# youmi-zym/TemporalStereo

Measured on AMD Instinct MI355X. Metric: stereo pairs/sec, FlyingThings3D 540x960 D=192 (aggregation hot path), higher is better.
Workload: dtype f32

## Files before the change

include/ts_hip.h:

```cpp
#ifndef TS_HIP_H
#define TS_HIP_H

#include <stddef.h>
#include <stdint.h>

#ifdef __cplusplus
extern "C" {
#endif

#define TS_OK 0
#define TS_ERR_NULL (-1)
#define TS_ERR_SHAPE (-2)
#define TS_ERR_UNSUPPORTED (-3)
#define TS_ERR_ALIGN (-4)

int ts_version(void);
const char* ts_last_error_string(void);

size_t ts_block_cost_workspace_bytes(int B, int C, int H, int W, int D, int scales);

int ts_block_cost_int_fwd(const float* left, const float* right, float* out, void* workspace,
                          int B, int C, int H, int W, int D, int scales, void* stream);

int ts_block_cost_sampled_fwd(const float* left, const float* right, const float* disp, float* out,
// ... 132 lines not shown
                          long long color_aug_stride, void* stream);
int ts_intrinsics_pyramid_fwd(const void* K_norm, int is_fp64, int B, int kh, int kw, int S, float* K, float* inv_K, void* stream);
int ts_disp_u16_decode_fwd(const void* raw, int B, int H, int W, float scale, float* disp, void* valid, void* stream);

#define TS_AUGMENT_ROW_INTS 96
#define TS_AUGMENT_MAX_RECTS 4
#define TS_AUGMENT_GAMMA 1
size_t ts_frames_augment_workspace_bytes(int B, int Hs, int Ws);
int ts_frames_augment_fwd(const void* left, const void* right, int B, int Hs, int Ws, int flags, float mean0, float mean1,
                          float mean2, float std0, float std1, float std2, int H, int W, const int* table, float* color_l,
                          float* color_r, long long color_stride, float* color_aug_l, float* color_aug_r,
                          long long color_aug_stride, void* workspace, size_t workspace_bytes, void* stream);
int ts_disp_u16_window_fwd(const void* raw, int B, int Hs, int Ws, int H, int W, const int* table, float scale, float* disp,
                           void* valid, void* stream);

int ts_topk_softargmax_fwd(const float* cost, const float* sample, const float* offset, float* disp,
                           float* topk_disp, float* topk_cost, int* topk_index,
                           int B, int D, int H, int W, int k, void* stream);

int ts_topk_softargmax_bwd(const float* topk_disp, const float* topk_cost, const int* topk_index,
                           const float* disp, const float* grad_disp, const float* grad_topk_disp,
                           const float* grad_topk_cost, float* grad_cost, float* grad_sample,
                           int B, int D, int H, int W, int k, void* stream);

int ts_softargmin_fwd(const float* cost, const float* sample, float* disp, float temperature,
                      int normalize, int B, int D, int H, int W, void* stream);

int ts_softargmin_bwd(const float* cost, const float* sample, const float* disp, const float* grad_disp,
                      float* grad_cost, float* grad_sample, float temperature, int normalize,
                      int B, int D, int H, int W, void* stream);

int ts_argmax_select_fwd(const float* cost, const float* sample, float* disp, int* index,
                         int B, int D, int H, int W, void* stream);

int ts_softsplat_sum_fwd(const float* input, const float* flow, float* output,
                         int B, int C, int H, int W, void* stream);
int ts_softsplat_sum_fwd_deterministic(const float* input, const float* flow, float* output, void* workspace,
                                       int B, int C, int H, int W, void* stream);
int ts_softsplat_sum_bwd_input(const float* flow, const float* grad_output, float* grad_input,
                               int B, int C, int H, int W, void* stream);
int ts_softsplat_sum_bwd_flow(const float* input, const float* flow, const float* grad_output,
                              float* grad_flow, int B, int C, int H, int W, void* stream);
size_t ts_softsplat_softmax_workspace_bytes(int B, int C, int H, int W);
int ts_softsplat_softmax_fwd(const float* input, const float* flow, const float* metric, float* output,
                             void* workspace, int B, int C, int H, int W, void* stream);
int ts_project_to_3d_fwd(const float* depth, const float* K, const float* inv_K, const float* T,
// ... 181 lines not shown
```

temporalstereo_amd/_lib.py:

```python
import ctypes
import os
import threading

_HERE = os.path.dirname(os.path.abspath(__file__))
LIB_PATH = os.path.join(_HERE, "libts_hip.so")

_lock = threading.Lock()
_lib = None

c_f32p = ctypes.c_void_p
c_ptr = ctypes.c_void_p
c_int = ctypes.c_int
c_size = ctypes.c_size_t
c_float = ctypes.c_float

SIGNATURES = {
    "ts_version": (c_int, []),
    "ts_last_error_string": (ctypes.c_char_p, []),
    "ts_block_cost_workspace_bytes": (c_size, [c_int] * 6),
    "ts_block_cost_int_fwd": (c_int, [c_f32p, c_f32p, c_f32p, c_ptr] + [c_int] * 6 + [c_ptr]),
    "ts_block_cost_sampled_fwd": (c_int, [c_f32p, c_f32p, c_f32p, c_f32p, c_ptr] + [c_int] * 6 + [c_ptr]),
    "ts_block_cost_sampled_warped_fwd": (c_int, [c_f32p, c_f32p, c_f32p, c_f32p, c_ptr] + [c_int] * 6 + [c_ptr]),
    "ts_block_cost_sampled_corr_fwd": (c_int, [c_f32p, c_f32p, c_f32p, c_f32p, c_ptr] + [c_int] * 6 + [c_ptr]),
    "ts_block_cost_corr_split_supported": (c_int, [c_int] * 2),
# ... 11 lines not shown
    "ts_cat_fms_fwd": (c_int, [c_f32p] * 4 + [c_int] * 5 + [c_ptr]),
    "ts_inverse_warp_3d_fwd": (c_int, [c_f32p] * 3 + [c_int] * 5 + [c_ptr]),
    "ts_dif_fms_workspace_bytes": (c_size, []),
    "ts_dif_fms_fwd": (c_int, [c_f32p] * 4 + [c_ptr] + [c_int] * 5 + [c_ptr]),
    "ts_correlation_fwd": (c_int, [c_f32p] * 3 + [c_int] * 7 + [c_ptr]),
    "ts_correlation_bwd": (c_int, [c_f32p] * 6 + [c_int] * 7 + [c_ptr]),
    "ts_block_cost_bwd_workspace_bytes": (c_size, [c_int] * 6),
    "ts_block_cost_int_bwd": (c_int, [c_f32p] * 5 + [c_ptr] + [c_int] * 6 + [c_ptr]),
    "ts_block_cost_sampled_bwd": (c_int, [c_f32p] * 7 + [c_ptr] + [c_int] * 6 + [c_ptr]),
    "ts_block_cost_sampled_warped_bwd": (c_int, [c_f32p] * 7 + [c_ptr] + [c_int] * 6 + [c_ptr]),
    "ts_calib_stream": (c_int, [c_int, c_ptr, c_ptr, c_size, c_ptr]),
    "ts_candidates_in_range_fwd": (c_int, [c_f32p] * 3 + [c_int] * 5 + [c_ptr]),
    "ts_candidates_in_range_bwd": (c_int, [c_f32p] * 5 + [c_int] * 5 + [c_ptr]),
    "ts_offset_head_fwd": (c_int, [c_f32p] * 2 + [ctypes.c_longlong, c_float, c_ptr]),
    "ts_offset_head_bwd": (c_int, [c_f32p] * 3 + [ctypes.c_longlong, c_float, c_ptr]),
    "ts_space_to_depth2_fwd": (c_int, [c_f32p] * 2 + [c_int] * 4 + [c_ptr]),
    "ts_deconv2d_k4s2_weight_to_conv3": (c_int, [c_f32p] * 2 + [c_int] * 3 + [c_ptr]),
    "ts_deconv2d_k4s2_wgrad_from_conv3": (c_int, [c_f32p] * 2 + [c_int] * 2 + [c_ptr]),
    "ts_bn_fold_many": (c_int, [c_ptr, c_int, c_float, c_ptr]),
    "ts_clip_rmsprop_workspace_bytes": (c_size, [c_int]),
    "ts_clip_rmsprop_step": (c_int, [c_ptr, c_int] + [c_float] * 4 + [c_ptr, c_size, c_ptr]),
    "ts_topk_softargmax_fwd": (c_int, [c_f32p] * 7 + [c_int] * 5 + [c_ptr]),
    "ts_topk_softargmax_bwd": (c_int, [c_f32p] * 9 + [c_int] * 5 + [c_ptr]),
    "ts_softargmin_fwd": (c_int, [c_f32p] * 3 + [c_float, c_int] + [c_int] * 4 + [c_ptr]),
    "ts_softargmin_bwd": (c_int, [c_f32p] * 6 + [c_float, c_int] + [c_int] * 4 + [c_ptr]),
    "ts_argmax_select_fwd": (c_int, [c_f32p] * 4 + [c_int] * 4 + [c_ptr]),
    "ts_bn_workspace_bytes": (c_size, [c_int, c_int, ctypes.c_longlong]),
    "ts_channel_splice_fwd": (c_int, [c_f32p] * 3 + [c_int] * 3 + [ctypes.c_longlong] * 4 + [c_ptr]),
    "ts_bn_sync_merge": (c_int, [c_f32p, c_int, c_int] + [c_f32p] * 4 + [c_float, c_f32p, c_ptr]),
    "ts_bn_train_fwd": (c_int, [c_f32p] * 5 + [c_float, c_ptr] + [c_f32p] * 3 + [c_ptr, c_int, c_int] + [ctypes.c_longlong] * 5 +
                        [c_float, c_int, c_ptr]),
    "ts_bn_train_bwd": (c_int, [c_f32p] * 9 + [c_ptr, c_int, c_int] + [ctypes.c_longlong] * 5 + [c_float, c_int, c_float, c_ptr]),
    "ts_bn_stats_fwd": (c_int, [c_f32p] * 5 + [c_float, c_ptr, c_ptr, c_int, c_int] + [ctypes.c_longlong] * 3 + [c_ptr]),
    "ts_bn_apply_act_fwd": (c_int, [c_f32p] * 6 + [c_int, c_int] + [ctypes.c_longlong] * 5 + [c_float, c_int, c_ptr]),
    "ts_bn_act_bwd_reduce": (c_int, [c_f32p] * 8 + [c_ptr, c_int, c_int] + [ctypes.c_longlong] * 5 + [c_float, c_int, c_ptr]),
    "ts_bn_act_bwd_apply": (c_int, [c_f32p] * 9 + [c_int, c_int] + [ctypes.c_longlong] * 5 + [c_float, c_int, c_int, c_float, c_ptr]),
    "ts_wasserstein_loss_workspace_bytes": (c_size, [c_int] * 3),
    "ts_wasserstein_loss_fwd": (c_int, [c_f32p] * 6 + [c_ptr] + [c_int] * 6 + [c_float, c_float, c_int, c_ptr]),
    "ts_wasserstein_loss_bwd": (c_int, [c_f32p] * 7 + [c_int] * 5 + [c_float, c_float, c_ptr]),
    "ts_disp_smooth_l1_workspace_bytes": (c_size, [c_int] * 3),
    "ts_disp_smooth_l1_fwd": (c_int, [c_f32p] * 3 + [c_ptr] + [c_int] * 5 + [c_float, c_float, c_ptr]),
    "ts_disp_smooth_l1_bwd": (c_int, [c_f32p] * 5 + [c_int] * 5 + [c_float, c_float, c_ptr]),
    "ts_disp_metrics_workspace_bytes": (c_size, [c_int] * 3),
    "ts_disp_metrics_fwd": (c_int, [c_f32p] * 4 + [c_int] * 9 + [c_f32p] * 2 + [c_int] * 3 + [c_float, c_float, c_int, c_f32p, c_ptr, c_ptr]),
    "ts_disp_render_workspace_bytes": (c_size, [c_int] * 3),
    "ts_disp_render_fwd": (c_int, [c_f32p] * 4 + [c_int] * 6 + [c_float] + [c_ptr] * 4 + [c_f32p, c_ptr, c_ptr]),
# ... 68 lines not shown
    "ts_resize_bilinear_pair_fwd": (c_int, [c_f32p] * 4 + [c_int] * 6 + [c_float, c_float, c_ptr]),
    "ts_range_candidates_fwd": (c_int, [c_f32p] * 4 + [c_int] * 3 + [c_float, c_int, c_int, c_ptr]),
    "ts_project_to_3d_fwd": (c_int, [c_f32p] * 7 + [c_int] * 6 + [c_float, c_ptr]),
    "ts_reproject_memory_workspace_bytes": (c_size, [c_int] * 5),
    "ts_reproject_memory_fwd": (c_int, [c_f32p, ctypes.c_longlong, c_int, c_int, c_f32p, c_f32p, c_int, c_f32p, c_int, c_int,
                                        c_f32p, c_int, c_f32p, c_f32p, c_f32p, c_float, c_float, c_f32p, c_f32p, c_f32p,
                                        c_ptr, c_int, c_int, c_int, c_ptr]),
    "ts_resize3d_add_act_bwd": (c_int, [c_f32p] * 5 + [c_int] * 9 + [c_ptr]),
    "ts_pool3d5_avgmax_bwd": (c_int, [c_f32p] * 4 + [c_int] * 5 + [c_ptr]),
    "ts_merge_candidates_bwd": (c_int, [c_f32p] * 5 + [c_int] * 5 + [c_ptr]),
    "ts_copy_rows_fwd": (c_int, [c_f32p] * 2 + [ctypes.c_longlong] * 4 + [c_ptr]),
    "ts_plan_create": (c_ptr, []),
    "ts_plan_destroy": (None, [c_ptr]),
    "ts_plan_length": (c_int, [c_ptr]),
    "ts_plan_add_call": (c_int, [c_ptr, ctypes.c_char_p, ctypes.POINTER(ctypes.c_ulonglong), c_int]),
    "ts_plan_run": (c_int, [c_ptr]),
    "ts_stream_fork": (c_int, [c_ptr, c_ptr]),
    "ts_event_record": (c_int, [c_int, c_ptr]),
    "ts_event_wait": (c_int, [c_int, c_ptr]),
}

_QUERIES = frozenset(n for n in SIGNATURES if n.endswith("_bytes") or n.startswith("ts_plan_") or
                     n.endswith("_split_supported") or
                     n in ("ts_version", "ts_last_error_string", "ts_conv_cout_pad", "ts_conv3d_hw_x6_supported", "ts_conv3d_hw_x6s_supported", "ts_peer_max_floats", "ts_peer_max_ranks",
                           "ts_peer_alloc", "ts_peer_open", "ts_peer_close", "ts_peer_free", "ts_peer_status", "ts_peer_status_async",
                           "ts_peer_set_timeout_ms", "ts_peer_reset", "ts_bn_set_small_elems",
                           "ts_conv_wgrad_defer", "ts_conv_wgrad_pending", "ts_conv_wgrad_take"))


def lib():
    rec = getattr(_tls, "recorder", None)
    if rec is not None:
        return rec.proxy
    return _real_lib()


def _real_lib():
    global _lib
    if _lib is None:
        with _lock:
            if _lib is None:
                if not os.path.exists(LIB_PATH):
                    raise RuntimeError(
                        "temporalstereo_amd: %s is missing -- build it with "
                        "`python -m temporalstereo_amd.build` (there is no fallback path)" % LIB_PATH)
                handle = ctypes.CDLL(LIB_PATH)
                for name, (res, args) in SIGNATURES.items():
# ... 115 lines not shown
```

temporalstereo_amd/aggregation/native.py:

```python
import os
import time

import torch
import torch.nn as nn

from .. import _lib
from .. import functional as TF

ACT_NONE, ACT_SILU, ACT_RELU, ACT_TANH_OFFSET, ACT_HEAD_PAIR = 0, 1, 2, 3, 4


def _stream():
    return _lib.current_stream_handle()


_PAR = {"on": False, "aux": None, "kinds": frozenset(__import__("os").environ.get("TS_BRANCHES", "hourglass").split(","))}


def _aux_stream():
    return _PAR["aux"]


_STAGE_CAP = int(os.environ.get("TS_STAGE_CHUNK_CAP", "8"))

# ... 414 lines not shown
        i2b, i2c = _strides5(split)
    assert Cin == f.cin, (Cin, f.cin)
    Dout = 2 * Din if transposed else (Din + 2 * padding - dilation * (k - 1) - 1) // stride + 1
    if out is None:
        out = torch.empty((B, f.cout, Dout, H, W), device=x.device, dtype=torch.float32)
    ib, ic = _strides5(x)
    ob, oc = _strides5(out)
    if split is not None:
        rc = _lib.lib().ts_conv3d_d_split_fwd(_lib.ptr(x), _lib.ptr(split), _lib.ptr(f.w), _lib.ptr(f.scale), _lib.ptr(f.shift),
                                              _lib.ptr(out), B, Cin, Cs, f.cout, Din, H, W, k, stride, dilation, padding,
                                              int(transposed), f.act if act is None else act, float(act_param),
                                              ib, ic, i2b, i2c, ob, oc, _stream())
        _lib.check(rc, "ts_conv3d_d_split_fwd")
        return out
    rc = _lib.lib().ts_conv3d_d_fwd(_lib.ptr(x), _lib.ptr(f.w), _lib.ptr(f.scale), _lib.ptr(f.shift), _lib.ptr(out),
                                    B, Cin, f.cout, Din, H, W, k, stride, dilation, padding, int(transposed),
                                    f.act if act is None else act, float(act_param), ib, ic, ob, oc, _stream())
    _lib.check(rc, "ts_conv3d_d_fwd")
    return out


FUSED_K1 = os.environ.get("TS_FUSED_K1", "1") != "0"
SPLIT_INPUT = os.environ.get("TS_SPLIT_INPUT", "1") != "0"


def block_cost_corr(left, right, disp, scales):
    return TF.block_cost_corr(left, right, disp, scales)


def conv_hw_warp(corr, f, q, disp, base, dilation=1):
    B, Cc, D, H, W = corr.shape
    assert Cc == f.cin, (Cc, f.cin)
    out = torch.empty((B, f.cout, D, H, W), device=corr.device, dtype=torch.float32)
    ib, ic = _strides5(corr)
    ob, oc = _strides5(out)
    wsb = TF._q("ts_conv3d_hw_warp_workspace_bytes", B, f.cout, D, H, W)
    ws = torch.empty(wsb, device=corr.device, dtype=torch.uint8)
    rc = _lib.lib().ts_conv3d_hw_warp_fwd(_lib.ptr(corr), _lib.ptr(f.w), _lib.ptr(f.scale), _lib.ptr(f.shift), _lib.ptr(out),
                                          _lib.ptr(q), _lib.ptr(disp), _lib.ptr(base), B, Cc, f.cout, D, H, W, dilation, f.act, 0.0,
                                          ib, ic, ob, oc, base.stride(0) if base is not None else 0, _lib.ptr(ws), wsb, _stream())
    _lib.check(rc, "ts_conv3d_hw_warp_fwd")
    return out


def resize_add_act(a, add, size, act=ACT_SILU):
    B, C, Da, Ha, Wa = a.shape
# ... 130 lines not shown
        f = object.__new__(Folded)
        f.cin, f.cout, f.kind, f.act, f.kshape = 2 * C, 2, "hw", ACT_HEAD_PAIR, self.c1.kshape
        pad = int(_lib.lib().ts_conv_cout_pad(2))
        f.w = torch.zeros(2 * C, self.c1.w.shape[1], pad, device=self.c1.w.device, dtype=torch.float32)
        f.w[:C, :, 0] = self.c1.w[:, :, 0]
        f.w[C:, :, 1] = self.o1.w[:, :, 0]
        f.scale = torch.ones(pad, device=f.w.device); f.shift = torch.zeros(pad, device=f.w.device)
        f.scale[0], f.scale[1] = self.c1.scale[0], self.o1.scale[0]
        f.shift[0], f.shift[1] = self.c1.shift[0], self.o1.shift[0]
        f._tape = _TAPE
        if _TAPE is not None:
            for k, (m, g) in enumerate(((mod.cost_head[1], self.c1), (mod.off_head[1], self.o1))):
                _TAPE.layout(f.w[k * C:(k + 1) * C], m.weight.detach(), False, col0=k)
                _TAPE.fold(f.scale[k:k + 1], f.shift[k:k + 1], m.bias, getattr(m, "norm", None), 1)
        self.pair = f

    def __call__(self, x):
        y = conv_d(x, self.co0, 3, 1, 1, 1)
        B, _, D, H, W = y.shape
        both = torch.empty((2, B, D, H, W), device=y.device, dtype=torch.float32)
        conv_hw(y, self.pair, out=both.permute(1, 0, 2, 3, 4), act_param=self.delta)
        return both[0], both[1]


class ConvexUp:

    def __init__(self, mod):
        self.r, self.k = mod.upscale_factor, mod.window_size
        if self.k != 3:
            raise NotImplementedError("window_size != 3")
        self.m0 = Folded(mod.mask[0].weight.unsqueeze(2), mod.mask[0].bias, mod.mask[1], ACT_SILU, False, "hw")
        w3 = mod.mask[3].weight
        self.m3 = Folded(w3.reshape(w3.shape[0], w3.shape[1], 1, 1, 1), mod.mask[3].bias, None, ACT_NONE, False, "d")

    def mask(self, feat):
        return conv_d(conv_hw(feat.unsqueeze(2), self.m0), self.m3, 1)

    def with_candidates(self, feat, disp, m, rng, extra_front=0):
        B, _, H, W = disp.shape
        if m is None:
            m = self.mask(feat)
        Ho, Wo = H * self.r, W * self.r
        out = torch.empty((B, 1, Ho, Wo), device=disp.device, dtype=torch.float32)
        low, high = torch.empty_like(out), torch.empty_like(out)
        cand = torch.empty((B, extra_front + 5, Ho, Wo), device=disp.device, dtype=torch.float32)
        disp = _lib.contiguous(disp)
# ... 78 lines not shown
        samp = torch.empty((B, Dm, H, W), device=vol.device, dtype=torch.float32)
        x0 = cat4[:, :C]
        vb, vc = _strides5(vol); ob, oc = _strides5(x0)
        rc = _lib.lib().ts_merge_candidates_fwd(_lib.ptr(vol), _lib.ptr(samples), _lib.ptr(mem_s), _lib.ptr(mem_c),
                                                _lib.ptr(self.past_w), _lib.ptr(self.past_scale), _lib.ptr(self.past_shift),
                                                _lib.ptr(samp), _lib.ptr(x0), B, C, D0, K, H, W, vb, vc, ob, oc, _stream())
        _lib.check(rc, "ts_merge_candidates_fwd")
        return cat4, samp

    def fuse(self, cat4):
        C = self.C
        x0 = cat4[:, :C]
        if not self.fusion:
            return x0
        br = Branch("pool")
        with br:
            pool5(x0, cat4[:, 2 * C:3 * C], cat4[:, 3 * C:])
        conv_d(x0, self.conv5, 5, 1, 1, 2, out=cat4[:, C:2 * C])
        br.join()
        return self.fuse_conv(cat4)

    def merge_fuse_predict(self, vol, samples, prev_info, feat, resize_memory, mask=None, next_range=None):
        cat4, samp = self.merge(vol, samples, prev_info, resize_memory)
        cost, off = self.heads(self.fuse(cat4))
        disp, _, _ = TF.topk_softargmax(cost, samp, off, k=self.topk)
        if callable(mask):
            mask = mask()
        if next_range is not None:
            return self.up.with_candidates(feat, disp, mask, *next_range), cost, off, samp
        return self.up(feat, disp, mask), cost, off, samp


class NativeCoarse(_MergingLevel):
    def early(self, left, right):
        return self.init3d(TF.block_cost(left, right, int(self.mod.num_sample), self.scales))

    def __call__(self, left, right, prev_info, mask=None, next_range=None, vol=None):
        if vol is None:
            vol = self.early(left, right)
        return self.merge_fuse_predict(vol, None, prev_info, left, resize_memory=True, mask=mask, next_range=next_range)


class NativeFine(_MergingLevel):
    def __init__(self, mod):
        super().__init__(mod)
        self.split_reference_half()

    def early(self, left, right, ds, terms=None):
# ... 107 lines not shown
        lcat, cat2, B, H, W = st
        f = self._c2d(self._c2d(lcat.unsqueeze(2), self.fuse[0], 1), self.fuse[1], 1).squeeze(2)
        self._deconv(_lib.contiguous(f), self.deconv4, cat2, cat2.stride(0))
        g = _lib.contiguous(self._c2d(cat2.unsqueeze(2), self.concat, 1).squeeze(2))
        mask = torch.empty((B, 9, 4 * H, 4 * W), device=lcat.device, dtype=torch.float32)
        self._deconv(g, self.deconv2, mask, mask.stride(0))
        return mask

    def early(self, both, lterm, ds):
        B = both.shape[0] // 2
        lcat, rcat = both.pair() if isinstance(both, SplitBoth) else (both[:B], both[B:])
        lt, rt = lterm
        if rt is not None:
            return self.init3d_from(self.first_layer_fused(lcat, rcat, ds, lt, rt))
        return self.init3d(TF.block_cost_warped(lcat, rcat, ds, self.scales), lt)

    def __call__(self, both, mask_lterm, ds, prev_info, vol=None):
        B = both.shape[0] // 2
        H, W = both.shape[-2:]
        mask, lterm = mask_lterm
        mask = mask() if callable(mask) else mask
        if vol is None:
            vol = self.early(both, lterm, ds)
        cost, off = self.heads(vol)
        disp, mem_s, mem_c = TF.topk_softargmax(cost, ds, off, k=self.topk)
        full = torch.empty((B, 1, 4 * H, 4 * W), device=both.device, dtype=torch.float32)
        rc = _lib.lib().ts_unet_upsample_fwd(_lib.ptr(mask), _lib.ptr(disp), _lib.ptr(full), B, H, W, 4 * H, 4 * W, _stream())
        _lib.check(rc, "ts_unet_upsample_fwd")
        prev_info['prev_disp'] = full
        mem_s, mem_c = resize_bilinear_pair(mem_s, mem_c, (H // 2, W // 2), 0.5, 1.0)
        prev_info['cost_memory'] = {'disp_sample': mem_s, 'cost_volume': mem_c}
        return full, disp, cost, off, ds


class NativeAggregator:

    def __init__(self, net, private_streams=False):
        if net.training:
            raise RuntimeError("NativeAggregator folds BatchNorm: put the module in eval() first")
        if any(p.device.type != "cuda" for p in net.parameters()):
            raise RuntimeError("NativeAggregator needs the module on the GPU (there is no CPU path)")
        dev = next(net.parameters()).device
        self.device = dev
        with torch.cuda.device(dev):
            self._build(net)
            torch.cuda.synchronize(dev)
        self.fast, self.aux = qualified_streams(dev, 2, private=private_streams)
        self._extra_streams = qualified_streams(dev, 3, private=True)
# ... 209 lines not shown
```

temporalstereo_amd/csrc/plan.hip:

```cpp
#include <cstdint>
#include <cstring>
#include <mutex>
#include <string>
#include <utility>
#include <vector>

#include "ts_common.hpp"

namespace {

constexpr int kMaxWords = 32;

template <class T>
T unpack(unsigned long long w) {
  static_assert(sizeof(T) <= sizeof(unsigned long long), "argument wider than a plan word");
  T v;
  std::memcpy(&v, &w, sizeof(T));
  return v;
}

template <class... A, size_t... I>
int call_with(int (*f)(A...), const unsigned long long* w, std::index_sequence<I...>) {
  return f(unpack<A>(w[I])...);
}
// ... 43 lines not shown
    TS_PLAN_OP(ts_disp_metrics_fwd),         TS_PLAN_OP(ts_disp_render_fwd),
    TS_PLAN_OP(ts_correlation_fwd),          TS_PLAN_OP(ts_correlation_bwd),
    TS_PLAN_OP(ts_bn_stats_fwd),             TS_PLAN_OP(ts_bn_apply_act_fwd),
    TS_PLAN_OP(ts_bn_act_bwd_reduce),        TS_PLAN_OP(ts_bn_act_bwd_apply),
    TS_PLAN_OP(ts_convex_upsample_bwd),      TS_PLAN_OP(ts_unet_upsample_bwd),
    TS_PLAN_OP(ts_conv_weight_layout),      TS_PLAN_OP(ts_conv_weight_layout_many),
    TS_PLAN_OP(ts_conv3d_hw_x6_fwd),        TS_PLAN_OP(ts_conv3d_hw_x6_weight_split), TS_PLAN_OP(ts_conv3d_hw_x6_weight_split_from),
    TS_PLAN_OP(ts_conv3d_hw_x6s_fwd),       TS_PLAN_OP(ts_conv3d_hw_x6s_weight_split),
    TS_PLAN_OP(ts_peer_all_gather),         TS_PLAN_OP(ts_peer_all_reduce_sum),
    TS_PLAN_OP(ts_bn_train_fwd),            TS_PLAN_OP(ts_bn_train_bwd),
    TS_PLAN_OP(ts_channel_splice_fwd),
    TS_PLAN_OP(ts_candidates_in_range_fwd), TS_PLAN_OP(ts_candidates_in_range_bwd),
    TS_PLAN_OP(ts_offset_head_fwd),         TS_PLAN_OP(ts_offset_head_bwd),
    TS_PLAN_OP(ts_space_to_depth2_fwd),
    TS_PLAN_OP(ts_deconv2d_k4s2_weight_to_conv3), TS_PLAN_OP(ts_deconv2d_k4s2_wgrad_from_conv3),
    TS_PLAN_OP(ts_clip_rmsprop_step),       TS_PLAN_OP(ts_bn_sync_merge),
    TS_PLAN_OP(ts_bn_fold_many),
    TS_PLAN_OP(ts_conv_weight_layout_many2), TS_PLAN_OP(ts_conv_wgrad_finish_many), TS_PLAN_OP(ts_channel_sum_fwd),
    TS_PLAN_OP(ts_block_cost_sampled_warped_bwd),
    TS_PLAN_OP(ts_frames_prepare_fwd),      TS_PLAN_OP(ts_intrinsics_pyramid_fwd),  TS_PLAN_OP(ts_disp_u16_decode_fwd),
    TS_PLAN_OP(ts_frames_augment_fwd),      TS_PLAN_OP(ts_disp_u16_window_fwd),
    TS_PLAN_OP(ts_block_cost_sampled_corr_split_fwd), TS_PLAN_OP(ts_conv3d_hw_split_fwd),
    TS_PLAN_OP(ts_conv3d_d_split_fwd),      TS_PLAN_OP(ts_conv3d_hw_x6_split_fwd),
};

struct Call {
  const Entry* op;
  unsigned long long w[kMaxWords];
};

__global__ void __launch_bounds__(256)
copy_rows_kernel(const float* __restrict__ src, float* __restrict__ dst, long long rows, long long row_elems,
                 long long src_pitch, long long dst_pitch) {
  const long long n = rows * row_elems;
  for (long long i = static_cast<long long>(blockIdx.x) * blockDim.x + threadIdx.x; i < n;
       i += static_cast<long long>(gridDim.x) * blockDim.x) {
    const long long r = i / row_elems, c = i - r * row_elems;
    dst[r * dst_pitch + c] = src[r * src_pitch + c];
  }
}

__global__ void __launch_bounds__(256)
copy_rows4_kernel(const float4* __restrict__ src, float4* __restrict__ dst, long long row_quads, long long src_pitch_q,
                  long long dst_pitch_q) {
  const float4* s = src + blockIdx.y * src_pitch_q;
  float4* d = dst + blockIdx.y * dst_pitch_q;
// ... 141 lines not shown
```

temporalstereo_amd/csrc/regress.hip:

```cpp
#include "ts_common.hpp"

namespace {

constexpr int KMAX = 8;

template <int K>
__global__ void __launch_bounds__(256)
topk_softargmax_fwd(const float* __restrict__ cost, const float* __restrict__ samp, const float* __restrict__ off,
                    float* __restrict__ disp, float* __restrict__ tdisp, float* __restrict__ tcost,
                    int* __restrict__ tidx, int B, int D, int HW) {
  const long long n = static_cast<long long>(B) * HW;
  for (long long i = static_cast<long long>(blockIdx.x) * blockDim.x + threadIdx.x; i < n;
       i += static_cast<long long>(gridDim.x) * blockDim.x) {
    const int b = static_cast<int>(i / HW);
    const int p = static_cast<int>(i - static_cast<long long>(b) * HW);
    const size_t base = static_cast<size_t>(b) * D * HW + p;
    float bc[K];
    int bi[K];
#pragma unroll
    for (int j = 0; j < K; ++j) { bc[j] = -INFINITY; bi[j] = -1; }
    for (int d0 = 0; d0 < D; d0 += 8) {
      float cc[8];
#pragma unroll
      for (int u = 0; u < 8; ++u) cc[u] = cost[base + static_cast<size_t>(min(d0 + u, D - 1)) * HW];
#pragma unroll
      for (int u = 0; u < 8; ++u) {
        float c = cc[u];
        int ci = d0 + u;
        const bool real = ci < D;
#pragma unroll
        for (int j = 0; j < K; ++j) {
          const bool take = real && ((c > bc[j]) || (bi[j] < 0));
          const float tc = bc[j];
          const int ti = bi[j];
          if (take) { bc[j] = c; bi[j] = ci; c = tc; ci = ti; }
        }
      }
    }
    float w[K], den = 0.f;
#pragma unroll
    for (int j = 0; j < K; ++j) { w[j] = expf(bc[j] - bc[0]); den += w[j]; }
    float acc = 0.f;
#pragma unroll
    for (int j = 0; j < K; ++j) {
      const size_t o = base + static_cast<size_t>(bi[j]) * HW;
      const float td = samp[o] + off[o];
      acc += (w[j] / den) * td;
      const size_t ko = (static_cast<size_t>(b) * K + j) * HW + p;
      tdisp[ko] = td;
      tcost[ko] = bc[j];
      if (tidx) tidx[ko] = bi[j];
    }
    disp[i] = acc;
  }
}

template <int K>
__global__ void __launch_bounds__(256)
topk_softargmax_bwd(const float* __restrict__ tdisp, const float* __restrict__ tcost, const int* __restrict__ tidx,
                    const float* __restrict__ disp, const float* __restrict__ gdisp, const float* __restrict__ gtd,
                    const float* __restrict__ gtc, float* __restrict__ gcost, float* __restrict__ gsamp,
                    int B, int D, int HW) {
  const long long n = static_cast<long long>(B) * HW;
  for (long long i = static_cast<long long>(blockIdx.x) * blockDim.x + threadIdx.x; i < n;
       i += static_cast<long long>(gridDim.x) * blockDim.x) {
    const int b = static_cast<int>(i / HW);
    const int p = static_cast<int>(i - static_cast<long long>(b) * HW);
    const size_t base = static_cast<size_t>(b) * D * HW + p;
    for (int d = 0; d < D; ++d) {
      if (gcost) gcost[base + static_cast<size_t>(d) * HW] = 0.f;
      if (gsamp) gsamp[base + static_cast<size_t>(d) * HW] = 0.f;
    }
    float c[K], td[K], w[K], den = 0.f;
    int idx[K];
#pragma unroll
    for (int j = 0; j < K; ++j) {
// ... 219 lines not shown
```

temporalstereo_amd/csrc/ts_common.hpp:

```cpp
#pragma once
#include <hip/hip_runtime.h>

#include <cstdarg>
#include <cstdint>
#include <cstdio>
#include <cstdlib>
#include <type_traits>

#include "../../include/ts_hip.h"

#define TS_ABI_VERSION 13

namespace ts {

char* err_buf();
int fail(int code, const char* fmt, ...);

inline hipStream_t as_stream(void* s) { return reinterpret_cast<hipStream_t>(s); }

inline bool aligned16(const void* p) { return (reinterpret_cast<uintptr_t>(p) & 15u) == 0; }

inline size_t round_up(size_t v, size_t a) { return (v + a - 1) / a * a; }

inline int launched(const char* what) {
  hipError_t e = hipGetLastError();
  if (e != hipSuccess) return fail(static_cast<int>(e), "%s: %s", what, hipGetErrorString(e));
  return TS_OK;
}

template <class F>
inline void dispatch_bool(bool b, F&& f) {
  if (b) f(std::true_type{});
  else f(std::false_type{});
}
// ... 23 lines not shown
```

temporalstereo_amd/functional.py:

```python
import torch

from . import _lib


def _stream():
    return _lib.current_stream_handle()


_QUERY = {}


def _q(name, *args):
    key = (name,) + args
    v = _QUERY.get(key)
    if v is None:
        v = _QUERY[key] = int(getattr(_lib._real_lib(), name)(*args))
    return v


_k1_probe = None


def _require_gpu(*tensors):
    dev = None
# ... 1535 lines not shown
        return disp, tdisp, tcost

    @staticmethod
    def backward(ctx, g_disp, g_tdisp, g_tcost):
        tdisp, tcost, tidx, disp = ctx.saved_tensors
        B, D, H, W, k = ctx.meta
        need_cost = ctx.needs_input_grad[0]
        need_samp = ctx.needs_input_grad[1] or ctx.needs_input_grad[2]
        gcost = torch.empty((B, D, H, W), device=disp.device, dtype=torch.float32) if need_cost else None
        gsamp = torch.empty((B, D, H, W), device=disp.device, dtype=torch.float32) if need_samp else None
        c = lambda t: None if t is None else _lib.contiguous(t)
        rc = _lib.lib().ts_topk_softargmax_bwd(_lib.ptr(tdisp), _lib.ptr(tcost), _lib.ptr(tidx), _lib.ptr(disp),
                                               _lib.ptr(c(g_disp)), _lib.ptr(c(g_tdisp)), _lib.ptr(c(g_tcost)),
                                               _lib.ptr(gcost), _lib.ptr(gsamp), B, D, H, W, k, _stream())
        _lib.check(rc, "ts_topk_softargmax_bwd")
        return (gcost, gsamp if ctx.needs_input_grad[1] else None,
                gsamp if ctx.needs_input_grad[2] else None, None)


def topk_softargmax(cost, disp_sample, off, k=2):
    return _TopkSoftArgmax.apply(cost, disp_sample, off, int(k))


class _SoftArgmin(torch.autograd.Function):
    @staticmethod
    def forward(ctx, cost, sample, temperature, normalize):
        _require_gpu(cost, sample)
        cost, sample = _lib.contiguous(cost), _lib.contiguous(sample)
        B, D, H, W = cost.shape
        disp = torch.empty((B, 1, H, W), device=cost.device, dtype=torch.float32)
        rc = _lib.lib().ts_softargmin_fwd(_lib.ptr(cost), _lib.ptr(sample), _lib.ptr(disp), float(temperature),
                                          int(bool(normalize)), B, D, H, W, _stream())
        _lib.check(rc, "ts_softargmin_fwd")
        ctx.save_for_backward(cost, sample, disp)
        ctx.meta = (B, D, H, W, float(temperature), int(bool(normalize)))
        return disp

    @staticmethod
    def backward(ctx, g):
        cost, sample, disp = ctx.saved_tensors
        B, D, H, W, temperature, normalize = ctx.meta
        gc = torch.empty_like(cost) if ctx.needs_input_grad[0] else None
        gs = torch.empty_like(sample) if ctx.needs_input_grad[1] else None
        g = _lib.contiguous(g)
        rc = _lib.lib().ts_softargmin_bwd(_lib.ptr(cost), _lib.ptr(sample), _lib.ptr(disp), _lib.ptr(g),
                                          _lib.ptr(gc), _lib.ptr(gs), temperature, normalize, B, D, H, W, _stream())
# ... 172 lines not shown
```

Measured before the change: 1553.

## Fuse head pair 3x3 conv with top-k soft-argmax regression in one kernel

Adds a kernel that computes the cost/offset head convolution over a tiled patch in shared memory and runs the top-k soft-argmax per pixel from shared memory in the same workgroup, replacing a separate conv_hw launch plus a topk_softargmax launch. This removes one launch and the re-read of the cost and offset volumes. It still writes cost and offset to global memory. The top-k routine moves into a shared header. The fused path only applies for small D (at most 16), C a multiple of 8 and a 1x3x3 kernel, and it may use the GPU less efficiently than the original tuned conv kernel.

```diff
diff --git a/include/ts_hip.h b/include/ts_hip.h
--- a/include/ts_hip.h
+++ b/include/ts_hip.h
@@ -178,6 +178,12 @@
                            const float* disp, const float* grad_disp, const float* grad_topk_disp,
                            const float* grad_topk_cost, float* grad_cost, float* grad_sample,
                            int B, int D, int H, int W, int k, void* stream);
+
+int ts_head_pair_topk_supported(int C, int D, int H, int W, int k);
+int ts_head_pair_topk_fwd(const float* y, const float* w, const float* scale, const float* shift, const float* sample,
+                          float* cost, float* off, float* disp, float* topk_disp, float* topk_cost, int* topk_index,
+                          int B, int C, int D, int H, int W, int k, int wpad, float delta, long long y_bstride,
+                          long long y_cstride, long long cost_bstride, long long off_bstride, void* stream);
 
 int ts_softargmin_fwd(const float* cost, const float* sample, float* disp, float temperature,
                       int normalize, int B, int D, int H, int W, void* stream);
diff --git a/temporalstereo_amd/_lib.py b/temporalstereo_amd/_lib.py
--- a/temporalstereo_amd/_lib.py
+++ b/temporalstereo_amd/_lib.py
@@ -57,6 +57,8 @@
     "ts_clip_rmsprop_step": (c_int, [c_ptr, c_int] + [c_float] * 4 + [c_ptr, c_size, c_ptr]),
     "ts_topk_softargmax_fwd": (c_int, [c_f32p] * 7 + [c_int] * 5 + [c_ptr]),
     "ts_topk_softargmax_bwd": (c_int, [c_f32p] * 9 + [c_int] * 5 + [c_ptr]),
+    "ts_head_pair_topk_supported": (c_int, [c_int] * 5),
+    "ts_head_pair_topk_fwd": (c_int, [c_f32p] * 11 + [c_int] * 7 + [c_float] + [ctypes.c_longlong] * 4 + [c_ptr]),
     "ts_softargmin_fwd": (c_int, [c_f32p] * 3 + [c_float, c_int] + [c_int] * 4 + [c_ptr]),
     "ts_softargmin_bwd": (c_int, [c_f32p] * 6 + [c_float, c_int] + [c_int] * 4 + [c_ptr]),
     "ts_argmax_select_fwd": (c_int, [c_f32p] * 4 + [c_int] * 4 + [c_ptr]),
@@ -171,7 +173,7 @@
 
 _QUERIES = frozenset(n for n in SIGNATURES if n.endswith("_bytes") or n.startswith("ts_plan_") or
                      n.endswith("_split_supported") or
-                     n in ("ts_version", "ts_last_error_string", "ts_conv_cout_pad", "ts_conv3d_hw_x6_supported", "ts_conv3d_hw_x6s_supported", "ts_peer_max_floats", "ts_peer_max_ranks",
+                     n in ("ts_version", "ts_last_error_string", "ts_conv_cout_pad", "ts_conv3d_hw_x6_supported", "ts_conv3d_hw_x6s_supported", "ts_head_pair_topk_supported", "ts_peer_max_floats", "ts_peer_max_ranks",
                            "ts_peer_alloc", "ts_peer_open", "ts_peer_close", "ts_peer_free", "ts_peer_status", "ts_peer_status_async",
                            "ts_peer_set_timeout_ms", "ts_peer_reset", "ts_bn_set_small_elems",
                            "ts_conv_wgrad_defer", "ts_conv_wgrad_pending", "ts_conv_wgrad_take"))
diff --git a/temporalstereo_amd/aggregation/native.py b/temporalstereo_amd/aggregation/native.py
--- a/temporalstereo_amd/aggregation/native.py
+++ b/temporalstereo_amd/aggregation/native.py
@@ -460,6 +460,7 @@
 
 FUSED_K1 = os.environ.get("TS_FUSED_K1", "1") != "0"
 SPLIT_INPUT = os.environ.get("TS_SPLIT_INPUT", "1") != "0"
+HEAD_FUSED = os.environ.get("TS_HEAD_FUSED", "1") != "0"
 
 
 def block_cost_corr(left, right, disp, scales):
@@ -636,6 +637,16 @@
         conv_hw(y, self.pair, out=both.permute(1, 0, 2, 3, 4), act_param=self.delta)
         return both[0], both[1]
 
+    def predict(self, x, samples, k):
+        y = conv_d(x, self.co0, 3, 1, 1, 1)
+        B, _, D, H, W = y.shape
+        both = torch.empty((2, B, D, H, W), device=y.device, dtype=torch.float32)
+        f = self.pair
+        if HEAD_FUSED and f.kshape == (1, 3, 3) and TF.head_pair_topk_supported(self.C, D, H, W, k):
+            return TF.head_pair_topk(y, f.w, f.scale, f.shift, samples, self.delta, k, cost=both[0], off=both[1])
+        conv_hw(y, f, out=both.permute(1, 0, 2, 3, 4), act_param=self.delta)
+        return (both[0], both[1]) + tuple(TF.topk_softargmax(both[0], samples, both[1], k=k))
+
 
 class ConvexUp:
 
@@ -760,8 +771,7 @@
 
     def merge_fuse_predict(self, vol, samples, prev_info, feat, resize_memory, mask=None, next_range=None):
         cat4, samp = self.merge(vol, samples, prev_info, resize_memory)
-        cost, off = self.heads(self.fuse(cat4))
-        disp, _, _ = TF.topk_softargmax(cost, samp, off, k=self.topk)
+        cost, off, disp, _, _ = self.heads.predict(self.fuse(cat4), samp, self.topk)
         if callable(mask):
             mask = mask()
         if next_range is not None:
@@ -915,8 +925,7 @@
         mask = mask() if callable(mask) else mask
         if vol is None:
             vol = self.early(both, lterm, ds)
-        cost, off = self.heads(vol)
-        disp, mem_s, mem_c = TF.topk_softargmax(cost, ds, off, k=self.topk)
+        cost, off, disp, mem_s, mem_c = self.heads.predict(vol, ds, self.topk)
         full = torch.empty((B, 1, 4 * H, 4 * W), device=both.device, dtype=torch.float32)
         rc = _lib.lib().ts_unet_upsample_fwd(_lib.ptr(mask), _lib.ptr(disp), _lib.ptr(full), B, H, W, 4 * H, 4 * W, _stream())
         _lib.check(rc, "ts_unet_upsample_fwd")
diff --git a/temporalstereo_amd/csrc/head_topk.hip b/temporalstereo_amd/csrc/head_topk.hip
--- /dev/null
+++ b/temporalstereo_amd/csrc/head_topk.hip
@@ -0,0 +1,175 @@
+#include "conv_common.hpp"
+#include "regress_topk.hpp"
+
+namespace {
+
+constexpr int kHeadChunk = 8;
+constexpr int kHeadThreads = 256;
+constexpr int kHeadMaxD = 16;
+
+struct HeadArgs {
+  const float* y;
+  const float* w;
+  const float* scale;
+  const float* shift;
+  const float* samp;
+  float* cost;
+  float* off;
+  float* disp;
+  float* tdisp;
+  float* tcost;
+  int* tidx;
+  int C, D, H, W, k, wpad;
+  float delta;
+  long long y_bs, y_cs, cost_bs, off_bs;
+  int tiles_x, tiles_y;
+};
+
+template <int TW, int TH, int DMAX>
+__global__ void __launch_bounds__(kHeadThreads)
+head_pair_topk_kernel(const HeadArgs a) {
+  constexpr int NPIX = TW * TH;
+  constexpr int PW = TW + 2, PH = TH + 2, PP = PW * PH;
+  constexpr int NSTAGE = kHeadChunk * DMAX * PP;
+  constexpr int NIT = (NSTAGE + kHeadThreads - 1) / kHeadThreads;
+  static_assert(NPIX * DMAX <= kHeadThreads, "one lane per (pixel, plane)");
+  __shared__ float sx[NSTAGE];
+  __shared__ float scost[DMAX * NPIX];
+  __shared__ float soff[DMAX * NPIX];
+
+  const int tid = threadIdx.x;
+  const int D = a.D, H = a.H, W = a.W, HW = H * W;
+  int t = blockIdx.x;
+  const int tx = t % a.tiles_x; t /= a.tiles_x;
+  const int ty = t % a.tiles_y;
+  const int b = t / a.tiles_y;
+  const int x0 = tx * TW, y0 = ty * TH;
+
+  const int nstage = kHeadChunk * D * PP;
+  int goff[NIT];
+  unsigned keep = 0;
+#pragma unroll
+  for (int i = 0; i < NIT; ++i) {
+    const int e = min(tid + i * kHeadThreads, nstage - 1);
+    const int plane = e / PP, r = e - plane * PP;
+    const int yy = r / PW, xx = r - yy * PW;
+    const int c = plane / D, d = plane - c * D;
+    const int gy = y0 + yy - 1, gx = x0 + xx - 1;
+    if (gy >= 0 && gy < H && gx >= 0 && gx < W) keep |= 1u << i;
+    goff[i] = c * static_cast<int>(a.y_cs) + d * HW + min(max(gy, 0), H - 1) * W + min(max(gx, 0), W - 1);
+  }
+  static_assert(NIT <= 32, "one mask bit per staging element");
+
+  const int p = tid % NPIX, dl = tid / NPIX;
+  const int px = p % TW, py = p / TW;
+  const int d = min(dl, D - 1);
+  const bool owns = dl < D && y0 + py < H && x0 + px < W;
+  const int lbase = (d * PH + py) * PW + px;
+
+  const float* yb = a.y + static_cast<size_t>(b) * a.y_bs;
+  const int nchunk = 2 * a.C / kHeadChunk;
+  float v[NIT];
+#pragma unroll
+  for (int i = 0; i < NIT; ++i) v[i] = yb[goff[i]];
+
+  float head[2] = {0.f, 0.f};
+  for (int ch = 0; ch < nchunk; ++ch) {
+    if (ch) __syncthreads();
+#pragma unroll
+    for (int i = 0; i < NIT; ++i) {
+      const int e = tid + i * kHeadThreads;
+      if (e < nstage) sx[e] = (keep >> i & 1u) ? v[i] : 0.f;
+    }
+    __syncthreads();
+    if (ch + 1 < nchunk) {
+      const float* yc = yb + static_cast<size_t>(ch + 1) * kHeadChunk * a.y_cs;
+#pragma unroll
+      for (int i = 0; i < NIT; ++i) v[i] = yc[goff[i]];
+    }
+    const int c0 = ch * kHeadChunk;
+    const int h = c0 >= a.C ? 1 : 0;
+    const float* wc = a.w + static_cast<size_t>(c0) * 9 * a.wpad + h;
+    float csum = 0.f;
+#pragma unroll
+    for (int c = 0; c < kHeadChunk; ++c) {
+      const float* xs = sx + c * D * PP + lbase;
+      float s = 0.f;
+#pragma unroll
+      for (int ky = 0; ky < 3; ++ky)
+#pragma unroll
+        for (int kx = 0; kx < 3; ++kx) s = fmaf(xs[ky * PW + kx], wc[(c * 9 + ky * 3 + kx) * a.wpad], s);
+      csum += s;
+    }
+    if (h) head[1] += csum;
+    else head[0] += csum;
+  }
+
+  const float vc = apply_act(head[0] * a.scale[0] + a.shift[0], ACT_HEAD_PAIR, a.delta, 0);
+  const float vo = apply_act(head[1] * a.scale[1] + a.shift[1], ACT_HEAD_PAIR, a.delta, 1);
+  if (dl < D) {
+    scost[dl * NPIX + p] = vc;
+    soff[dl * NPIX + p] = vo;
+  }
+  if (owns) {
+    const size_t o = static_cast<size_t>(d) * HW + static_cast<size_t>(y0 + py) * W + (x0 + px);
+    a.cost[static_cast<size_t>(b) * a.cost_bs + o] = vc;
+    a.off[static_cast<size_t>(b) * a.off_bs + o] = vo;
+  }
+  __syncthreads();
+
+  if (tid < NPIX && y0 + py < H && x0 + px < W) {
+    const size_t pix = static_cast<size_t>(y0 + py) * W + (x0 + px);
+    const float* sp = a.samp + static_cast<size_t>(b) * D * HW + pix;
+    float* dp = a.disp + static_cast<size_t>(b) * HW + pix;
+    const size_t ko = static_cast<size_t>(b) * a.k * HW + pix;
+#define TS_CASE(KK)                                                                                               \
+  case KK:                                                                                                        \
+    topk_softargmax_pixel<KK>(scost + p, NPIX, sp, HW, soff + p, NPIX, D, dp, a.tdisp + ko, a.tcost + ko,          \
+                              a.tidx ? a.tidx + ko : nullptr, HW);                                                \
+    break;
+    switch (a.k) { TS_CASE(1) TS_CASE(2) TS_CASE(3) TS_CASE(4) TS_CASE(5) TS_CASE(6) TS_CASE(7) TS_CASE(8) }
+#undef TS_CASE
+  }
+}
+
+bool head_supported(int C, int D, int H, int W, int k) {
+  return C > 0 && C % kHeadChunk == 0 && D >= 1 && D <= kHeadMaxD && H > 0 && W > 0 && k >= 1 && k <= KMAX && k <= D &&
+         static_cast<long long>(kHeadChunk) * D * H * W < (1ll << 31);
+}
+
+}
+
+extern "C" int ts_head_pair_topk_supported(int C, int D, int H, int W, int k) { return head_supported(C, D, H, W, k) ? 1 : 0; }
+
+extern "C" int ts_head_pair_topk_fwd(const float* y, const float* w, const float* scale, const float* shift, const float* sample,
+                                     float* cost, float* off, float* disp, float* topk_disp, float* topk_cost, int* topk_index,
+                                     int B, int C, int D, int H, int W, int k, int wpad, float delta, long long y_bstride,
+                                     long long y_cstride, long long cost_bstride, long long off_bstride, void* stream) {
+  TS_REQUIRE(B > 0 && C > 0 && D > 0 && H > 0 && W > 0, TS_ERR_SHAPE, "head_pair_topk: non-positive size");
+  TS_REQUIRE(k >= 1 && k <= KMAX && k <= D, TS_ERR_UNSUPPORTED, "head_pair_topk: k=%d outside 1..min(%d, D=%d)", k, KMAX, D);
+  TS_REQUIRE(D <= kHeadMaxD, TS_ERR_UNSUPPORTED, "head_pair_topk: D=%d planes, one workgroup holds %d", D, kHeadMaxD);
+  TS_REQUIRE(C % kHeadChunk == 0, TS_ERR_UNSUPPORTED, "head_pair_topk: C=%d is not a multiple of %d", C, kHeadChunk);
+  TS_REQUIRE(head_supported(C, D, H, W, k), TS_ERR_UNSUPPORTED, "head_pair_topk: channel volume too large");
+  TS_REQUIRE(wpad >= 2, TS_ERR_SHAPE, "head_pair_topk: weight pitch %d holds no two columns", wpad);
+  const long long vol = static_cast<long long>(D) * H * W;
+  TS_REQUIRE(y_cstride >= vol && y_bstride >= 0 && cost_bstride >= vol && off_bstride >= vol, TS_ERR_SHAPE,
+             "head_pair_topk: a stride is shorter than a channel's planes");
+  TS_REQUIRE(kHeadChunk * y_cstride < (1ll << 31), TS_ERR_UNSUPPORTED, "head_pair_topk: channel stride too large");
+  TS_REQUIRE_PTR(y); TS_REQUIRE_PTR(w); TS_REQUIRE_PTR(scale); TS_REQUIRE_PTR(shift); TS_REQUIRE_PTR(sample);
+  TS_REQUIRE_PTR(cost); TS_REQUIRE_PTR(off); TS_REQUIRE_PTR(disp); TS_REQUIRE_PTR(topk_disp); TS_REQUIRE_PTR(topk_cost);
+  HeadArgs a{y, w, scale, shift, sample, cost, off, disp, topk_disp, topk_cost, topk_index, C, D, H, W, k, wpad, delta,
+             y_bstride, y_cstride, cost_bstride, off_bstride, 0, 0};
+  hipStream_t st = ts::as_stream(stream);
+  auto launch = [&](auto kern, int tw, int th) {
+    a.tiles_x = (W + tw - 1) / tw;
+    a.tiles_y = (H + th - 1) / th;
+    const long long blocks = static_cast<long long>(a.tiles_x) * a.tiles_y * B;
+    if (blocks >= (1ll << 31)) return ts::fail(TS_ERR_UNSUPPORTED, "head_pair_topk: grid too large");
+    hipLaunchKernelGGL(kern, dim3(static_cast<unsigned>(blocks)), dim3(kHeadThreads), 0, st, a);
+    return ts::launched("head_pair_topk_fwd");
+  };
+  if (D <= 4) return launch(head_pair_topk_kernel<16, 4, 4>, 16, 4);
+  if (D <= 5) return launch(head_pair_topk_kernel<16, 3, 5>, 16, 3);
+  if (D <= 8) return launch(head_pair_topk_kernel<8, 4, 8>, 8, 4);
+  return launch(head_pair_topk_kernel<8, 2, 16>, 8, 2);
+}
diff --git a/temporalstereo_amd/csrc/plan.hip b/temporalstereo_amd/csrc/plan.hip
--- a/temporalstereo_amd/csrc/plan.hip
+++ b/temporalstereo_amd/csrc/plan.hip
@@ -89,6 +89,7 @@
     TS_PLAN_OP(ts_frames_augment_fwd),      TS_PLAN_OP(ts_disp_u16_window_fwd),
     TS_PLAN_OP(ts_block_cost_sampled_corr_split_fwd), TS_PLAN_OP(ts_conv3d_hw_split_fwd),
     TS_PLAN_OP(ts_conv3d_d_split_fwd),      TS_PLAN_OP(ts_conv3d_hw_x6_split_fwd),
+    TS_PLAN_OP(ts_head_pair_topk_fwd),
 };
 
 struct Call {
diff --git a/temporalstereo_amd/csrc/regress.hip b/temporalstereo_amd/csrc/regress.hip
--- a/temporalstereo_amd/csrc/regress.hip
+++ b/temporalstereo_amd/csrc/regress.hip
@@ -1,8 +1,6 @@
-#include "ts_common.hpp"
+#include "regress_topk.hpp"
 
 namespace {
-
-constexpr int KMAX = 8;
 
 template <int K>
 __global__ void __launch_bounds__(256)
@@ -15,43 +13,9 @@
     const int b = static_cast<int>(i / HW);
     const int p = static_cast<int>(i - static_cast<long long>(b) * HW);
     const size_t base = static_cast<size_t>(b) * D * HW + p;
-    float bc[K];
-    int bi[K];
-#pragma unroll
-    for (int j = 0; j < K; ++j) { bc[j] = -INFINITY; bi[j] = -1; }
-    for (int d0 = 0; d0 < D; d0 += 8) {
-      float cc[8];
-#pragma unroll
-      for (int u = 0; u < 8; ++u) cc[u] = cost[base + static_cast<size_t>(min(d0 + u, D - 1)) * HW];
-#pragma unroll
-      for (int u = 0; u < 8; ++u) {
-        float c = cc[u];
-        int ci = d0 + u;
-        const bool real = ci < D;
-#pragma unroll
-        for (int j = 0; j < K; ++j) {
-          const bool take = real && ((c > bc[j]) || (bi[j] < 0));
-          const float tc = bc[j];
-          const int ti = bi[j];
-          if (take) { bc[j] = c; bi[j] = ci; c = tc; ci = ti; }
-        }
-      }
-    }
-    float w[K], den = 0.f;
-#pragma unroll
-    for (int j = 0; j < K; ++j) { w[j] = expf(bc[j] - bc[0]); den += w[j]; }
-    float acc = 0.f;
-#pragma unroll
-    for (int j = 0; j < K; ++j) {
-      const size_t o = base + static_cast<size_t>(bi[j]) * HW;
-      const float td = samp[o] + off[o];
-      acc += (w[j] / den) * td;
-      const size_t ko = (static_cast<size_t>(b) * K + j) * HW + p;
-      tdisp[ko] = td;
-      tcost[ko] = bc[j];
-      if (tidx) tidx[ko] = bi[j];
-    }
-    disp[i] = acc;
+    const size_t ko = static_cast<size_t>(b) * K * HW + p;
+    topk_softargmax_pixel<K>(cost + base, HW, samp + base, HW, off + base, HW, D, disp + i, tdisp + ko, tcost + ko,
+                             tidx ? tidx + ko : nullptr, HW);
   }
 }
 
diff --git a/temporalstereo_amd/csrc/regress_topk.hpp b/temporalstereo_amd/csrc/regress_topk.hpp
--- /dev/null
+++ b/temporalstereo_amd/csrc/regress_topk.hpp
@@ -0,0 +1,50 @@
+#pragma once
+#include "ts_common.hpp"
+
+namespace {
+
+constexpr int KMAX = 8;
+
+template <int K>
+__device__ __forceinline__ void topk_softargmax_pixel(const float* __restrict__ cost, size_t cs, const float* __restrict__ samp, size_t ss,
+                                                      const float* __restrict__ off, size_t os, int D, float* __restrict__ disp,
+                                                      float* __restrict__ tdisp, float* __restrict__ tcost, int* __restrict__ tidx,
+                                                      size_t ks) {
+  float bc[K];
+  int bi[K];
+#pragma unroll
+  for (int j = 0; j < K; ++j) { bc[j] = -INFINITY; bi[j] = -1; }
+  for (int d0 = 0; d0 < D; d0 += 8) {
+    float cc[8];
+#pragma unroll
+    for (int u = 0; u < 8; ++u) cc[u] = cost[static_cast<size_t>(min(d0 + u, D - 1)) * cs];
+#pragma unroll
+    for (int u = 0; u < 8; ++u) {
+      float c = cc[u];
+      int ci = d0 + u;
+      const bool real = ci < D;
+#pragma unroll
+      for (int j = 0; j < K; ++j) {
+        const bool take = real && ((c > bc[j]) || (bi[j] < 0));
+        const float tc = bc[j];
+        const int ti = bi[j];
+        if (take) { bc[j] = c; bi[j] = ci; c = tc; ci = ti; }
+      }
+    }
+  }
+  float w[K], den = 0.f;
+#pragma unroll
+  for (int j = 0; j < K; ++j) { w[j] = expf(bc[j] - bc[0]); den += w[j]; }
+  float acc = 0.f;
+#pragma unroll
+  for (int j = 0; j < K; ++j) {
+    const float td = samp[static_cast<size_t>(bi[j]) * ss] + off[static_cast<size_t>(bi[j]) * os];
+    acc += (w[j] / den) * td;
+    tdisp[j * ks] = td;
+    tcost[j * ks] = bc[j];
+    if (tidx) tidx[j * ks] = bi[j];
+  }
+  *disp = acc;
+}
+
+}
diff --git a/temporalstereo_amd/csrc/ts_common.hpp b/temporalstereo_amd/csrc/ts_common.hpp
--- a/temporalstereo_amd/csrc/ts_common.hpp
+++ b/temporalstereo_amd/csrc/ts_common.hpp
@@ -9,7 +9,7 @@
 
 #include "../../include/ts_hip.h"
 
-#define TS_ABI_VERSION 13
+#define TS_ABI_VERSION 14
 
 namespace ts {
 
diff --git a/temporalstereo_amd/functional.py b/temporalstereo_amd/functional.py
--- a/temporalstereo_amd/functional.py
+++ b/temporalstereo_amd/functional.py
@@ -1581,6 +1581,36 @@
     return _TopkSoftArgmax.apply(cost, disp_sample, off, int(k))
 
 
+def head_pair_topk_supported(C, D, H, W, k):
+    return bool(_q("ts_head_pair_topk_supported", int(C), int(D), int(H), int(W), int(k)))
+
+
+def head_pair_topk(y, w, scale, shift, disp_sample, delta, k=2, cost=None, off=None, want_index=False):
+    _require_gpu(y, w, scale, shift, disp_sample)
+    B, C2, D, H, W = y.shape
+    if y.stride(4) != 1 or y.stride(3) != W or y.stride(2) != H * W:
+        raise ValueError("head_pair_topk: y's planes must be dense")
+    if tuple(disp_sample.shape) != (B, D, H, W) or w.shape[0] != C2 or w.shape[1] != 9 or C2 % 2:
+        raise ValueError("head_pair_topk: y [B,2C,D,H,W], w [2C,9,pad], disp_sample [B,D,H,W]")
+    disp_sample = _lib.contiguous(disp_sample)
+    dev = y.device
+    cost = torch.empty((B, D, H, W), device=dev, dtype=torch.float32) if cost is None else cost
+    off = torch.empty((B, D, H, W), device=dev, dtype=torch.float32) if off is None else off
+    for t in (cost, off):
+        if tuple(t.shape) != (B, D, H, W) or not t[0].is_contiguous():
+            raise ValueError("head_pair_topk: cost / off must be [B,D,H,W] with dense batch elements")
+    disp = torch.empty((B, 1, H, W), device=dev, dtype=torch.float32)
+    tdisp = torch.empty((B, k, H, W), device=dev, dtype=torch.float32)
+    tcost = torch.empty_like(tdisp)
+    tidx = torch.empty((B, k, H, W), device=dev, dtype=torch.int32) if want_index else None
+    rc = _lib.lib().ts_head_pair_topk_fwd(_lib.ptr(y), _lib.ptr(w), _lib.ptr(scale), _lib.ptr(shift), _lib.ptr(disp_sample),
+                                          _lib.ptr(cost), _lib.ptr(off), _lib.ptr(disp), _lib.ptr(tdisp), _lib.ptr(tcost),
+                                          _lib.ptr(tidx), B, C2 // 2, D, H, W, int(k), w.shape[2], float(delta),
+                                          y.stride(0), y.stride(1), cost.stride(0), off.stride(0), _stream())
+    _lib.check(rc, "ts_head_pair_topk_fwd")
+    return (cost, off, disp, tdisp, tcost) + ((tidx,) if want_index else ())
+
+
 class _SoftArgmin(torch.autograd.Function):
     @staticmethod
     def forward(ctx, cost, sample, temperature, normalize):
```

After: 1472. 0.948x the previous value.
